# CTPLab/Tera-MIND

Hardware: AMD Instinct MI355X
Metric: denoising steps/sec on 64x64x(2 stains x 2 z) patches (interior patch-steps/s) (higher is better)
Workload: dtype f32; 1 GPU; configs[1]: b=32 images x 1 interior 64x64 patch (P=1, 128 padded + 32 collage patches/step), rna_slc=4, rna_num=229, stain=all, DDPM T=50 schedule, f32, mode A (pad+patchify -> UNet -> DDPM update); parallelism=dp1 (independent patch batches)

## Files before the change

### include/teramind_hip.h

```cpp
#ifndef TERAMIND_HIP_H
#define TERAMIND_HIP_H

#include <stddef.h>
#include <stdint.h>

#ifdef __cplusplus
extern "C" {
#endif

#define TM_ABI_VERSION 1

enum {
  TM_OK = 0,
  TM_ERR_ARG = -1,
  TM_ERR_STATE = -2,
  TM_ERR_KEY = -3,
  TM_ERR_HIP = -4,
  TM_ERR_WORKSPACE = -5
};

enum { TM_DTYPE_F32 = 0, TM_DTYPE_BF16 = 1, TM_DTYPE_F16 = 2 };
enum { TM_SAMPLE_DDPM = 0, TM_SAMPLE_DDIM = 1 };

typedef struct tm_config {
// ... 154 lines not shown
                        int res_half, int N, int Cin, int Cout, int Z, int S, int ksize, int zmode, int up2,
                        int tile_variant, void* stream);

int tm_op_conv_zpair_fused_f32(const void* x_cb8, const void* w_host, const void* bias_host, const void* norm_w_host,
                               const void* scale_host, const void* shift_host, const void* res_cb8, void* a2_out,
                               void* h1_out, void* a2_sep_out, int N, int Cin, int Cout, int Z, int S, int per_image,
                               int tile_variant, void* stream);

int tm_op_conv_ups_pair_f32(const void* x_cb8, const void* w_host, const void* bias_host, void* y_cb8, int N, int Cin,
                            int Cout, int Z, int S, int tile_variant, void* stream);

int tm_op_conv_xpair_f32(const void* x_cb8, const void* w_host, const void* bias_host, void* y_cb8, const void* res_cb8,
                         int res_half, int N, int Cin, int Cout, int Z, int S, int tile_variant, void* stream);
int tm_op_conv_xquad_f32(const void* x_cb8, const void* w_host, const void* bias_host, void* y_cb8, const void* res_cb8,
                         int res_half, int N, int Cin, int Cout, int Z, int S, int tile_variant, void* stream);
int tm_op_conv_pad1_time_f32(const void* x_cb8, const void* w_host, const void* bias_host, void* y_cb8, int N, int Cin,
                             int Cout, int S, int form, int tile_variant, int iters, float* ms_out, void* stream);

int tm_op_conv1_f32(const void* x_cb8, const void* w_host, const void* bias_host, void* y_cb8, const void* res_cb8,
                    const void* gate_cb8, int x_cbtot, int x_cb0, int gate_cbtot, int gate_cb0, int gate_half, int gelu,
                    int tile_variant, int N, int Cin, int Cout, int Z, int S, int* form_out, void* stream);
int tm_conv1_form(long vox, int ntile, int tile_variant);

int tm_conv_frag_addrs(int kernel, int half, int tw, int what, int wave, int p, int ky, int kx, int sub, int* out64);

int tm_op_conv27_bf16(const void* x_cb8, const void* w_host, const void* bias_host, void* y_cb8,
                      int N, int Cin, int Cout, int S, int dtype, int waves, const void* res_h16, void* y_h16,
                      int ups, int res_half, void* stream);
int tm_op_conv27_h16_z(const void* x_cb8, const void* w_host, const void* bias_host, void* y_cb8,
                       int N, int Cin, int Cout, int S, int dtype, int waves, const void* res_h16, void* y_h16,
                       int ups, int res_half, int Z, void* stream);

// ... 135 lines not shown
```

### tera-mind_amd/_lib.py

```python
import ctypes as C
import os

_HERE = os.path.dirname(os.path.abspath(__file__))
LIB_PATH = os.environ.get("TM_LIB_PATH") or os.path.join(_HERE, "csrc", "libteramind_hip.so")

c_void_p, c_int, c_size_t, c_char_p, c_float = C.c_void_p, C.c_int, C.c_size_t, C.c_char_p, C.c_float
c_i64_p = C.POINTER(C.c_int64)


class TmConfig(C.Structure):
    _fields_ = [("patch_size", C.c_int32), ("rna_slc", C.c_int32), ("n_stain", C.c_int32),
                ("rna_num", C.c_int32), ("net_ch", C.c_int32), ("ch_mult", C.c_int32 * 4),
                ("embed_ch", C.c_int32), ("attn_res", C.c_int32), ("num_res_blocks", C.c_int32),
                ("vis_only", C.c_int32), ("dtype", C.c_int32)]


class TmStepCoefs(C.Structure):
    _fields_ = [("sqrt_recip_alphas_cumprod", c_float), ("sqrt_recipm1_alphas_cumprod", c_float),
                ("posterior_mean_coef1", c_float), ("posterior_mean_coef2", c_float),
                ("sigma", c_float), ("sqrt_alpha_bar_prev", c_float),
                ("sqrt_one_minus_alpha_bar_prev", c_float)]


class TmProfStats(C.Structure):
# ... 61 lines not shown
    "tm_op_to_cb8": (c_int, [c_void_p, c_void_p, c_int, c_int, c_int, c_int, c_int, c_void_p]),
    "tm_op_from_cb8": (c_int, [c_void_p, c_void_p, c_int, c_int, c_int, c_int, c_int, c_void_p]),
    "tm_op_conv_mfma": (c_int, [c_void_p, c_void_p, c_void_p, c_void_p] + [c_int] * 9 + [c_void_p]),
    "tm_op_conv_mfma_res": (c_int, [c_void_p, c_void_p, c_void_p, c_void_p, c_void_p] + [c_int] * 10 + [c_void_p]),
    "tm_op_conv1_f32": (c_int, [c_void_p] * 6 + [c_int] * 12 + [C.POINTER(c_int), c_void_p]),
    "tm_conv1_form": (c_int, [C.c_long, c_int, c_int]),
    "tm_conv_frag_addrs": (c_int, [c_int] * 9 + [c_void_p]),
    "tm_op_conv27_bf16": (c_int, [c_void_p, c_void_p, c_void_p, c_void_p] + [c_int] * 6 + [c_void_p] * 2 + [c_int] * 2 + [c_void_p]),
    "tm_op_conv27_fused": (c_int, [c_void_p] * 7 + [c_int] * 7 + [c_void_p]),
    "tm_op_conv27_h16_z": (c_int, [c_void_p, c_void_p, c_void_p, c_void_p] + [c_int] * 6 + [c_void_p] * 2 + [c_int] * 3 + [c_void_p]),
    "tm_op_conv27_fused_z": (c_int, [c_void_p] * 7 + [c_int] * 8 + [c_void_p]),
    "tm_op_conv_zpair_fused_f32": (c_int, [c_void_p] * 10 + [c_int] * 7 + [c_void_p]),
    "tm_op_conv_ups_pair_f32": (c_int, [c_void_p] * 4 + [c_int] * 6 + [c_void_p]),
    "tm_op_conv_xpair_f32": (c_int, [c_void_p] * 5 + [c_int] * 7 + [c_void_p]),
    "tm_op_conv_xquad_f32": (c_int, [c_void_p] * 5 + [c_int] * 7 + [c_void_p]),
    "tm_op_conv_pad1_time_f32": (c_int, [c_void_p] * 4 + [c_int] * 7 + [C.POINTER(c_float), c_void_p]),
    "tm_op_conv27_time":(c_int, [c_int] * 10 + [c_void_p, c_void_p]),
    "tm_op_conv1_bf16": (c_int, [c_void_p, c_void_p, c_void_p, c_void_p] + [c_int] * 8 + [c_void_p] * 4),
    "tm_op_conv1_h16_gate": (c_int, [c_void_p, c_void_p, c_void_p, c_void_p] + [c_int] * 8 + [c_void_p] * 3 + [c_int] * 3 + [c_void_p]),
    "tm_op_conv1_concat": (c_int, [c_void_p, c_void_p, c_void_p, c_int, c_void_p, c_void_p, c_void_p] + [c_int] * 8 + [c_void_p]),
    "tm_op_prep_h16": (c_int, [c_void_p] * 3 + [c_int] * 7 + [c_void_p, c_int, c_int, c_void_p, c_void_p, C.c_long] +
                       [c_int] * 4 + [c_void_p, c_void_p, c_int, c_void_p, c_void_p]),
    "tm_op_prep_f32": (c_int, [c_void_p] * 3 + [c_int] * 7 + [c_void_p, c_int, c_int, c_void_p, c_void_p, C.c_long] +
                       [c_int] * 4 + [c_void_p, c_void_p, c_int, c_void_p, c_void_p]),
    "tm_op_prep_form": (c_int, [c_void_p] * 3 + [c_int] * 9 + [c_void_p, c_int, c_int, c_int, c_void_p, c_void_p, C.c_long] +
                        [c_int] * 5 + [c_void_p, c_void_p, c_int, c_int, c_void_p, c_void_p]),
    "tm_op_stem": (c_int, [c_void_p] * 4 + [c_int] * 6 + [c_void_p]),
    "tm_op_head": (c_int, [c_void_p] * 4 + [c_int] * 6 + [c_void_p]),
    "tm_op_time_embed": (c_int, [c_void_p] * 7 + [c_int] * 3 + [c_void_p]),
    "tm_op_emb_all": (c_int, [c_void_p] * 4 + [c_int] * 3 + [c_void_p]),
    "tm_op_prep_train": (c_int, [c_void_p] * 5 + [c_float, c_int, c_void_p] + [c_int] * 4 + [c_void_p]),
# ... 68 lines not shown
```

### tera-mind_amd/csrc/tm_kernels.h

```cpp
#pragma once
#include <hip/hip_runtime.h>
#include <stdint.h>

#include <vector>

#include "../../include/teramind_hip.h"

namespace tmk {

struct TV {
  float* p = nullptr;
  int N = 0, C = 0, Cb = 0, Z = 0, H = 0, W = 0;
  long nstride = 0;
  long plane() const { return (long)Z * H * W * 8; }
  TV blocks(int cb0, int ncb) const {
    TV v = *this;
    v.p = p + (long)cb0 * plane();
    v.Cb = ncb;
    v.C = ncb * 8;
    return v;
  }
};
inline TV cb8_view(void* p, int N, int C, int Z, int H, int W) {
  TV t;
// ... 38 lines not shown

enum { EPI_NONE = 0, EPI_GELU = 1, EPI_UP2 = 2 };
enum { ZM_PAD1 = 0, ZM_INPLANE = 1, ZM_VALID = 2,
       ZM_UPS = 3 };
struct ConvLaunch {
  TV x;
  ConvW w;
  TV y;
  const TV* res = nullptr;
  const TV* gate = nullptr;
  int flags = 0;
  int tile_variant = 0;
  int gate_half = 0;
  int res_half = 0;
  int zmode = ZM_PAD1;
  int fuse_norm = 0;
  const float *norm_w = nullptr, *mod_scale = nullptr, *mod_shift = nullptr;
  float inv_c = 0.f;
  long mod_stride = 0;
  int per_image = 1;
  TV a2;
};
hipError_t launch_conv_mfma(const ConvLaunch& L, hipStream_t s);
int conv_tile(int form, long ovox, int ntile, int S, int tile_variant);
int conv_frag_addrs(int kernel, int half, int tw, int what, int wv, int p, int ky, int kx, int sub, int* out);
int conv1_form(long vox, int ntile, int tile_variant);

struct TVH {
  uint16_t* p = nullptr;
  int N = 0, C = 0, Cb = 0, Z = 0, H = 0, W = 0;
  long nstride = 0;
  TVH blocks(int cb0, int ncb) const {
    TVH t = *this;
    t.p = p + (long)cb0 * Z * H * W * 8;
    t.Cb = ncb; t.C = ncb * 8;
    return t;
  }
};
struct ConvLaunchH {
  TVH x;
// ... 298 lines not shown
```

### tera-mind_amd/csrc/tm_kernels.hip

```cpp
#include "tm_conv_pair.h"

#include <stdlib.h>
#include <string.h>

#include <type_traits>

namespace tmk {

template <int NZI, int WM, int TW, bool UPS = false>
struct C3Geo {
  static constexpr int TW_ = TW;
  static constexpr int MV = 4 * WM * 32;
  static constexpr int TR = (MV / TW < TW) ? (MV / TW) : TW;
  static constexpr int NPB = MV / (TR * TW);
  static constexpr int HR = TR + 2, HC = TW + 2;
  static constexpr int XV = NPB * NZI * HR * HC;
  static constexpr int XPIECES = XV * 2;
  static constexpr int PX = (XPIECES + 255) / 256;
  static constexpr int TZ = UPS ? 4 : 9;
  static constexpr int NTAP = TZ * NZI;
  static constexpr int WFLOATS = NTAP * 512;
  static constexpr int WPIECES = WFLOATS / 4;
  static constexpr int PW = (WPIECES + 255) / 256;
  static constexpr int TAPS_TOTAL = (NZI == 1) ? 9 : 3 * TZ;
// ... 638 lines not shown
    }
#pragma unroll
    for (int z = 0; z < 2; ++z)
#pragma unroll
      for (int par = 0; par < 2; ++par) {
        f32x16 o[1][1];
        o[0][0] = acc[0][par] + acc[1 + z][par];
        asm volatile("" : "+v"(o[0][0]));
        const int ooff[1] = {ooff0 >= 0 ? ooff0 + (z * S * S + par) * 8 : -1};
        __builtin_amdgcn_sched_barrier(0);
        conv_epilogue<1, 1>(a, o, nte, h, on, ooff, 2 * S);
      }
  }
}

template <int HALF, int TW>
struct XQGeo {
  static constexpr int TW_ = TW;
  static constexpr int NW = HALF ? 4 : 8;
  static constexpr int MG = 16 * NW;
  static constexpr int GW = TW / 4;
  static constexpr int TR = (MG / GW < TW) ? (MG / GW) : TW;
  static constexpr int NPB = MG / (TR * GW);
  static constexpr int HR = TR + 2;
  static constexpr int XP = NPB * HR * GW;
  static constexpr int XITEMS = XP * 2;
  static_assert(XP % 8 == 0, "whole groups of eight staging items (tm_conv_frag.h)");
  static constexpr int WTAP = 256;
  static constexpr int WSLOT = 18 * WTAP;
  static constexpr int KP = (18 + NW - 1) / NW;
  static constexpr int LDS_BYTES = (2 * WSLOT + 18 * XP * 8) * 4;
  static_assert(2 * WSLOT * 4 <= 65536 && LDS_BYTES <= 160 * 1024, "LDS-DMA destinations below 64 KiB, the CU's LDS");
};
TM_HD constexpr int xq_lane_group(int tw, int i32) { return tw == 8 ? conv_lane_voxel(16, i32) : i32; }
template <class G>
TM_HD constexpr int xq_xtap(int q, int ky) { return q * G::XP * 8 + conv_frag_off(ky * G::GW, 0, G::XP); }

template <int HALF, int TW>
__global__ __launch_bounds__(HALF ? 256 : 512, 2) void conv3d_xquad(ConvArgs a) {
  using G = XQGeo<HALF, TW>;
  static_assert(G::XITEMS <= 64 * G::NW, "one staging item per thread");
  extern __shared__ __attribute__((aligned(16))) float lds[];
  float* lw = lds;

  const int tid = threadIdx.x;
  const int lane = tid & 63, wv = tid >> 6;
  const int i32 = lane & 31, h = lane >> 5;

  const int S = a.S;
  const ConvTile t = conv_tile_of<TW, G::TR, false, false>(a);
  const int nt = t.nt, pg = t.pg, tr = t.tr, tc = t.tc;

  long xoff = -1;
  bool okl = false, okr = false;
  if (tid < G::XITEMS) {
    const int half = conv_stage_half(tid);
    int v = conv_stage_row(tid);
    const int j = v % G::GW; v /= G::GW;
    const int hr = v % G::HR;
    const int ps = v / G::HR;
    const int n = pg * G::NPB + ps;
    const int y = tr * G::TR + hr - 1, x = tc * TW + 4 * j;
    if (n < a.N && y >= 0 && y < S) {
      xoff = (long)n * a.x_nstride + ((long)y * S + x) * 8 + half * 4;
      okl = x > 0;
      okr = x + 4 < S;
    }
  }
  const long zplane = (long)S * S * 8;
  int xw = 2 * G::WSLOT + conv_frag_off(conv_stage_row(tid), conv_stage_half(tid), G::XP);
  asm volatile("" : "+v"(xw));

  const int gt = wv >> 1;
  const int qh = wv & 1;
  int xb[3], on[1], ooff0;
  {
    const ConvLane l = conv_lane_of<G::TR, G::GW, G::HR * G::GW, G::GW, G::XP>(gt * 32 + xq_lane_group(TW, i32), h, 0, 0);
#pragma unroll
    for (int p = 0; p < 3; ++p) {
      xb[p] = (2 * G::WSLOT + (p * 6 + 3 * qh) * G::XP * 8 + l.xb) / 4;
      asm volatile("" : "+v"(xb[p]));
    }
    const int n = pg * G::NPB + l.ps;
    on[0] = n;
    const int y = tr * G::TR + l.r, x = tc * TW + 4 * l.c;
    ooff0 = n < a.N ? (y * S + x) * 8 : -1;
  }
  const int wb = 3 * qh * G::WTAP + conv_frag_off(i32, h, 32);

  f32x16 acc[3][3];
  clear_acc(acc);

  const unsigned lw_lds = (unsigned)(size_t)(__attribute__((address_space(3))) float*)lw;
  const rsrc_words wrs = weight_rsrc<true>(a.w + (long)nt * a.Cbi * 3 * G::WSLOT, a.Cbi * 3 * G::WSLOT * 4);
  const int wvo = lane * 16;
// ... 4 lines not shown

  f32x4 xr[2][6];
  const f32x4 zero4 = {0.f, 0.f, 0.f, 0.f};
  auto load_x = [&](int cb) {
    const float* xp = a.x + (long)cb * a.x_plane;
#pragma unroll
    for (int z = 0; z < 2; ++z) {
      const float* b = xp + xoff + z * zplane;
      xr[z][0] = okl ? *(const f32x4*)(b - 8) : zero4;
#pragma unroll
      for (int c = 0; c < 4; ++c) xr[z][1 + c] = xoff >= 0 ? *(const f32x4*)(b + 8 * c) : zero4;
      xr[z][5] = okr ? *(const f32x4*)(b + 32) : zero4;
    }
  };
  auto put_t = [&](int p, const f32x4 (&d)[6]) __attribute__((always_inline)) {
    float* o = lds + xw + p * 6 * G::XP * 8;
    const f32x4 e42 = d[4] - d[2];
    *(f32x4*)(o) = (4.f * d[0] - 5.f * d[2]) + d[4];
    *(f32x4*)(o + G::XP * 8) = (d[3] + d[4]) - 4.f * (d[1] + d[2]);
    *(f32x4*)(o + 2 * G::XP * 8) = 4.f * (d[1] - d[2]) - (d[3] - d[4]);
    *(f32x4*)(o + 3 * G::XP * 8) = 2.f * (d[3] - d[1]) + e42;
    *(f32x4*)(o + 4 * G::XP * 8) = 2.f * (d[1] - d[3]) + e42;
    *(f32x4*)(o + 5 * G::XP * 8) = (4.f * d[1] - 5.f * d[3]) + d[5];
  };

  load_x(0);
#pragma unroll
  for (int k = 0; k < G::KP; ++k) issue_piece(0, k);
  auto stage = [&](int cb, auto more_c) __attribute__((always_inline)) {
    constexpr bool more = decltype(more_c)::value;
    asm volatile("s_waitcnt vmcnt(0)" ::: "memory");
    __builtin_amdgcn_s_barrier();
    asm volatile("" ::: "memory");
    if (tid < G::XITEMS) {
      put_t(2, xr[0]);
#pragma unroll
      for (int c = 0; c < 6; ++c) xr[0][c] = xr[0][c] + xr[1][c];
      put_t(0, xr[0]);
      put_t(1, xr[1]);
    }
// ... 20 lines not shown
      for (int ky = 0; ky < 3; ++ky) {
#pragma unroll
        for (int q = 0; q < 3; ++q) {
          const f32x4 wf = *(const f32x4*)(lwc + (ky * 6 + q) * G::WTAP);
          const f32x4 xf = ((const f32x4*)lds)[xb[p] + xq_xtap<G>(q, ky) / 4];
#pragma unroll
          for (int kk = 0; kk < 4; ++kk) acc[p][q] = __builtin_amdgcn_mfma_f32_32x32x2f32(wf[kk], xf[kk], acc[p][q], 0, 0, 0);
          if (ky * 3 + q < G::KP && (p < 2 || more)) issue_piece(n + 1, ky * 3 + q);
        }
      }
    }
    __builtin_amdgcn_s_setprio(0);
  };
  for (int cb = 0; cb + 1 < a.Cbi; ++cb) stage(cb, std::true_type{});
  stage(a.Cbi - 1, std::false_type{});

  const int qhu = __builtin_amdgcn_readfirstlane(qh);
#pragma unroll
  for (int p = 0; p < 3; ++p) {
    if (qhu) {
      const f32x16 sp = acc[p][0] + acc[p][1];
      acc[p][0] = acc[p][0] - acc[p][1];
      acc[p][1] = sp;
    } else {
      const f32x16 s = acc[p][1] + acc[p][2];
      acc[p][2] = acc[p][1] - acc[p][2];
      acc[p][1] = s;
    }
    asm volatile("" : "+v"(acc[p][0]), "+v"(acc[p][1]), "+v"(acc[p][2]));
  }
// ... 151 lines not shown
static bool conv_fills_chip(long vox, long tiles) { return (vox / 256) * tiles >= 512; }

int conv1_form(long vox, int ntile, int tile_variant) {
  if (tile_variant == 3) return (ntile & 1) == 0 ? 3 : 0;
  const int variant = tile_variant ? tile_variant : (conv_fills_chip(vox, ntile) ? 2 : 1);
  if (variant == 2 && (ntile & 1) == 0 && conv_fills_chip(vox, ntile / 2)) return 3;
  return variant == 2 ? 2 : 1;
}

int conv_tile(int form, long ovox, int ntile, int S, int tile_variant) {
  if (S == 4) return 1;
  if (form == CF_XQUAD) return tile_variant ? (tile_variant == 2 ? 2 : 1) : ((ovox / 1024) * 2 * ntile >= 256 ? 2 : 1);
  const long tiles = (form == CF_ZSKIP_UPS || form == CF_PAIR_UPS) ? 4L * ntile : ntile;
  const int variant = tile_variant ? tile_variant : (conv_fills_chip(ovox, tiles) ? 2 : 1);
  return variant == 2 ? 2 : 1;
}

template <void (*KERN)(ConvArgs), class G, int BLOCK = 256>
static hipError_t launch_tiled(const ConvArgs& a, long factor, hipStream_t s) {
  static DevOnce attr_once;
  if (attr_once.need()) {
    hipError_t e = hipFuncSetAttribute((const void*)KERN, hipFuncAttributeMaxDynamicSharedMemorySize, G::LDS_BYTES);
    if (e != hipSuccess) return e;
    attr_once.mark();
  }
  const long tiles = (long)(a.S / G::TW_) * (a.S / G::TR);
  const long pgs = (a.N + G::NPB - 1) / G::NPB;
  hipLaunchKernelGGL(KERN, dim3((unsigned)(pgs * tiles * factor * a.ntile)), dim3(BLOCK), G::LDS_BYTES, s, a);
  return hipGetLastError();
}
// ... 104 lines not shown
      return with_tile_width<32>(S, [&](auto tw) {
        constexpr int TW = decltype(tw)::value;
        if (L.fuse_norm) return launch_tiled<conv3d_zpair<0, TW, true>, ZPGeo<0, TW>>(a, 1, s);
        return large ? launch_tiled<conv3d_zpair<0, TW, false>, ZPGeo<0, TW>>(a, 1, s)
                     : launch_tiled<conv3d_zpair<1, TW, false>, ZPGeo<1, TW>>(a, 1, s);
      });
    case CF_PAIR_UPS:
      if (S == 4) return launch_tiled<conv3d_zpair_ups<1, 4>, ZPUGeo<1, 4>>(a, 4, s);
      return with_tile_width<32>(S, [&](auto tw) {
        constexpr int TW = decltype(tw)::value;
        return large ? launch_tiled<conv3d_zpair_ups<0, TW>, ZPUGeo<0, TW>>(a, 4, s)
                     : launch_tiled<conv3d_zpair_ups<1, TW>, ZPUGeo<1, TW>>(a, 4, s);
      });
    case CF_XQUAD:
      a.ntile = (L.w.Cout + 31) / 32;
      return with_tile_width<16>(S, [&](auto tw) {
        constexpr int TW = decltype(tw)::value;
        return large ? launch_tiled<conv3d_xquad<0, TW>, XQGeo<0, TW>, 64 * XQGeo<0, TW>::NW>(a, 1, s)
                     : launch_tiled<conv3d_xquad<1, TW>, XQGeo<1, TW>, 64 * XQGeo<1, TW>::NW>(a, 1, s);
      });
    default:
      return with_tile_width<16>(S, [&](auto tw) {
        constexpr int TW = decltype(tw)::value;
        return large ? launch_tiled<conv3d_xpair<0, TW>, XPGeo<0, TW>, 64 * XPGeo<0, TW>::NW>(a, 1, s)
                     : launch_tiled<conv3d_xpair<1, TW>, XPGeo<1, TW>, 64 * XPGeo<1, TW>::NW>(a, 1, s);
      });
  }
}

template <class G, int HALF, int TW, bool UPS>
static int zpair_frag_addrs(int what, int wv, int p, int ky, int kx, int sub, int* out) {
  constexpr int NC = HALF ? 1 : 2, KW = UPS ? 2 : 3;
  constexpr int lx = G::LDS_BYTES / 4 - 3 * G::XV * 8;
  if (p < 0 || p > 2) return -1;
// ... 19 lines not shown
  using G = XPGeo<HALF, TW>;
  if (p < 0 || p > 2 || q < 0 || q >= (what == 2 ? 4 : G::NQ) || ky < 0 || ky > (what == 2 ? 0 : 2)) return -1;
  const int pt = HALF ? 0 : (wv >> 1), ch = wv & 1, q0 = HALF ? (wv >> 1) * 2 : 0;
  for (int lane = 0; lane < 64; ++lane) {
    const int i32 = lane & 31, h = lane >> 5, tid = wv * 64 + lane;
    int a = -1;
    if (what == 0) a = q0 * 512 + conv_w_off(ch * 32 + i32, 4 * h) + (ky * 4 + q) * 512;
    else if (what == 1)
      a = 2 * G::WSLOT + q0 * G::XP * 8 + conv_lane_of<G::TR, G::PWD, G::HR * G::PWD, G::PWD, G::XP>(pt * 32 + i32, h, 0, 0).xb + xp_xtap<G>(p, q, ky);
    else if (tid < G::XITEMS)
      a = 2 * G::WSLOT + conv_frag_off(conv_stage_row(tid), conv_stage_half(tid), G::XP) + (p * 4 + q) * G::XP * 8;
    out[lane] = a < 0 ? -1 : a * 4;
  }
  return 0;
}
template <int HALF, int TW>
static int xquad_frag_addrs(int what, int wv, int p, int ky, int q, int* out) {
  using G = XQGeo<HALF, TW>;
  if (wv >= G::NW || p < 0 || p > 2 || q < 0 || q >= (what == 2 ? 6 : 3) || ky < 0 || ky > (what == 2 ? 0 : 2)) return -1;
  const int gt = wv >> 1, qh = wv & 1;
  for (int lane = 0; lane < 64; ++lane) {
    const int i32 = lane & 31, h = lane >> 5, tid = wv * 64 + lane;
    int a = -1;
    if (what == 0) a = 3 * qh * G::WTAP + conv_frag_off(i32, h, 32) + (ky * 6 + q) * G::WTAP;
    else if (what == 1)
      a = 2 * G::WSLOT + (p * 6 + 3 * qh) * G::XP * 8 +
          conv_lane_of<G::TR, G::GW, G::HR * G::GW, G::GW, G::XP>(gt * 32 + xq_lane_group(TW, i32), h, 0, 0).xb + xq_xtap<G>(q, ky);
    else if (tid < G::XITEMS)
      a = 2 * G::WSLOT + conv_frag_off(conv_stage_row(tid), conv_stage_half(tid), G::XP) + (p * 6 + q) * G::XP * 8;
    out[lane] = a < 0 ? -1 : a * 4;
  }
  return 0;
}
int conv_frag_addrs(int kernel, int half, int tw, int what, int wv, int p, int ky, int kx, int sub, int* out) {
  if (!out || kernel < 0 || kernel > 4 || kernel == 3 || half < 0 || half > 1 || what < 0 || what > 2 || wv < 0 || wv > (kernel == 4 ? 7 : 3)) return -1;
  if (kernel == 4 && tw == 8) return half ? xquad_frag_addrs<1, 8>(what, wv, p, ky, kx, out) : xquad_frag_addrs<0, 8>(what, wv, p, ky, kx, out);
  if (kernel == 4 && tw == 16) return half ? xquad_frag_addrs<1, 16>(what, wv, p, ky, kx, out) : xquad_frag_addrs<0, 16>(what, wv, p, ky, kx, out);
  if (kernel == 4) return -1;
#define TM_FRAG(H, T)                                                                                              \
  if (half == H && tw == T) {                                                                                      \
    if (kernel == 0) return zpair_frag_addrs<ZPGeo<H, T>, H, T, false>(what, wv, p, ky, kx, sub, out);              \
    if (kernel == 1) return zpair_frag_addrs<ZPUGeo<H, T>, H, T, true>(what, wv, p, ky, kx, sub, out);              \
  }
  TM_FRAG(1, 4) TM_FRAG(0, 8) TM_FRAG(1, 8) TM_FRAG(0, 16) TM_FRAG(1, 16) TM_FRAG(0, 32) TM_FRAG(1, 32)
#undef TM_FRAG
  if (kernel == 2 && tw == 8) return half ? xpair_frag_addrs<1, 8>(what, wv, p, ky, kx, out) : xpair_frag_addrs<0, 8>(what, wv, p, ky, kx, out);
  if (kernel == 2 && tw == 16) return half ? xpair_frag_addrs<1, 16>(what, wv, p, ky, kx, out) : xpair_frag_addrs<0, 16>(what, wv, p, ky, kx, out);
  return -1;
}

struct PrepArgs { PrepLaunch L; };
struct PrepDropArgs { PrepLaunch L; DropRng r; };
__device__ __forceinline__ DropRng rng_of(const PrepArgs&) { return DropRng{0ull, 0u, 0u}; }
// ... 970 lines not shown
```

### tera-mind_amd/csrc/tm_ops.hip

```cpp
#include "../../include/teramind_hip.h"
#include "tm_kernels.h"

#include <algorithm>
#include <cmath>
#include <cstdint>
#include <tuple>
#include <utility>
#include <vector>
#include <string.h>

using namespace tmk;

struct DevTmp {
  std::vector<void*> ptrs;
  std::vector<hipEvent_t> events;
  hipError_t err = hipSuccess;
  const char* what = "";
  bool ordered = false;
  hipStream_t st = nullptr;
  DevTmp() = default;
  explicit DevTmp(hipStream_t stream) : ordered(true), st(stream) { keep_pool(); }
  static void keep_pool() {
    static bool done[64] = {};
    int dev = 0;
// ... 232 lines not shown
  const int rc = finish((hipStream_t)stream, launch_conv_mfma(op.L, (hipStream_t)stream), "conv_xpair (fp32)");
  return rc ? rc : conv_tile(CF_XPAIR, (long)N * Z * S * S, op.L.w.ntile, S, tile_variant);
}

static int xquad_args(const void* x, const void* w, const void* b, const void* y, int N, int Cin, int Cout, int Z, int S,
                      int tile_variant) {
  if (!x || !w || !b || !y) return fail(TM_ERR_ARG, "null argument");
  if (N < 1 || Cin < 1 || Cout < 1) return fail(TM_ERR_ARG, "N, Cin, Cout must be positive");
  if (Z != 2) return fail(TM_ERR_ARG, "the x-quad form exists at Z == 2 only (got Z = %d)", Z);
  if (S != 8 && S != 16 && S != 32 && S != 64 && S != 128) return fail(TM_ERR_ARG, "S must be 8, 16, 32, 64 or 128 (got %d)", S);
  if (tile_variant < 0 || tile_variant > 2) return fail(TM_ERR_ARG, "tile_variant must be 0 (auto), 1 or 2 (got %d)", tile_variant);
  if (conv_pick_form(3, ZM_PAD1, 2, true, ROLE_OP_XQUAD) != CF_XQUAD)
    return fail(TM_ERR_ARG, "the x-quad form is switched off (TM_CONV_XQUAD=0)");
  return TM_OK;
}
extern "C" int tm_op_conv_xquad_f32(const void* x_cb8, const void* w_host, const void* bias_host, void* y_cb8, const void* res_cb8,
                                    int res_half, int N, int Cin, int Cout, int Z, int S, int tile_variant, void* stream) {
  if (const int rc = xquad_args(x_cb8, w_host, bias_host, y_cb8, N, Cin, Cout, Z, S, tile_variant)) return rc;
  if (res_half && !res_cb8) return fail(TM_ERR_ARG, "res_half needs a residual");
  ConvOp op;
  if (const int rc = conv_op(op, CF_XQUAD, w_host, bias_host, x_cb8, y_cb8, N, Cin, Cout, Z, S, Z, S, ZM_PAD1, tile_variant, res_cb8,
                             res_half))
    return rc;
  const int rc = finish((hipStream_t)stream, launch_conv_mfma(op.L, (hipStream_t)stream), "conv_xquad (fp32)");
  return rc ? rc : conv_tile(CF_XQUAD, (long)N * Z * S * S, op.L.w.ntile, S, tile_variant);
}

extern "C" int tm_op_conv_pad1_time_f32(const void* x_cb8, const void* w_host, const void* bias_host, void* y_cb8, int N, int Cin,
                                        int Cout, int S, int form, int tile_variant, int iters, float* ms_out, void* stream) {
  if (const int rc = form == 2 ? xquad_args(x_cb8, w_host, bias_host, y_cb8, N, Cin, Cout, 2, S, tile_variant)
                               : xpair_args(x_cb8, w_host, bias_host, y_cb8, N, Cin, Cout, 2, S, tile_variant))
    return rc;
  if (form < 0 || form > 2 || iters < 1 || !ms_out) return fail(TM_ERR_ARG, "form must be 0, 1 or 2, iters >= 1, ms_out non-null");
  const int cf = conv_pick_form(3, ZM_PAD1, 2, true, form == 2 ? ROLE_OP_XQUAD : form ? ROLE_OP_XPAIR : ROLE_OP);
  if (!form && cf != CF_PAIR) return fail(TM_ERR_ARG, "the pair form is switched off (TM_CONV_ZPAIR=0)");
  ConvOp op;
  if (const int rc = conv_op(op, cf, w_host, bias_host, x_cb8, y_cb8, N, Cin, Cout, 2, S, 2, S, ZM_PAD1, tile_variant)) return rc;
  hipEvent_t e0 = op.tmp.event(), e1 = op.tmp.event();
  if (op.tmp.err) return op.tmp.report();
  hipStream_t st = (hipStream_t)stream;
  for (int i = 0; i < iters; ++i) {
    HIP_TRY(hipEventRecord(e0, st));
    HIP_TRY(launch_conv_mfma(op.L, st));
    HIP_TRY(hipEventRecord(e1, st));
    HIP_TRY(hipEventSynchronize(e1));
    HIP_TRY(hipEventElapsedTime(ms_out + i, e0, e1));
  }
  return finish(st, hipSuccess, "conv_pad1_time (fp32)");
}

static bool half_gate_ok(int S) { return S >= 2 && (S & (S - 1)) == 0; }

extern "C" int tm_conv1_form(long vox, int ntile, int tile_variant) { return conv1_form(vox, ntile, tile_variant); }
extern "C" int tm_conv_frag_addrs(int kernel, int half, int tw, int what, int wave, int p, int ky, int kx, int sub, int* out64) {
  return conv_frag_addrs(kernel, half, tw, what, wave, p, ky, kx, sub, out64);
}

extern "C" int tm_op_conv1_f32(const void* x_cb8, const void* w_host, const void* bias_host, void* y_cb8, const void* res_cb8,
                               const void* gate_cb8, int x_cbtot, int x_cb0, int gate_cbtot, int gate_cb0, int gate_half, int gelu,
                               int tile_variant, int N, int Cin, int Cout, int Z, int S, int* form_out, void* stream) {
  if (!x_cb8 || !w_host || !bias_host || !y_cb8) return fail(TM_ERR_ARG, "null argument");
  if (N < 1 || Cin < 1 || Cout < 1 || Z < 1 || S < 1) return fail(TM_ERR_ARG, "N, Cin, Cout, Z, S must be positive");
  const int Cbi = (Cin + 7) / 8, Cob = (Cout + 7) / 8;
  if (x_cb0 < 0 || x_cb0 + Cbi > x_cbtot)
    return fail(TM_ERR_ARG, "x slice: blocks [%d, %d) run past the %d blocks of the tensor", x_cb0, x_cb0 + Cbi, x_cbtot);
  if (gate_half && !gate_cb8) return fail(TM_ERR_ARG, "gate_half without a gate");
  if (gate_half && !half_gate_ok(S)) return fail(TM_ERR_ARG, "gate_half: S must be a power of two >= 2 (got %d)", S);
  if (gate_cb8 && (gate_cb0 < 0 || gate_cb0 + Cob > gate_cbtot))
// ... 1248 lines not shown
```

Measured before the change: 996.8 interior patch-steps/s.

## Add software-pipelined schedule to x-quad Winograd conv kernel with double-buffered staging

Adds a PIPE variant of the x-quad 3D conv kernel that double-buffers the transformed input sets and weight slots in LDS. The next channel block's global loads, Winograd transforms and LDS-DMA weight pieces are interleaved with the current block's MFMA taps, so only one barrier is needed per z-plane step instead of several. The aim is to hide load and staging latency behind matrix math. It becomes the default for the large tile at width 16, with an env switch to turn it off, and it costs more register pressure and a more complex waitcnt schedule.

New measurement: 1011 interior patch-steps/s, median of 6. 1.5% higher.

```diff
diff --git a/include/teramind_hip.h b/include/teramind_hip.h
--- a/include/teramind_hip.h
+++ b/include/teramind_hip.h
@@ -192,8 +192,13 @@
                          int res_half, int N, int Cin, int Cout, int Z, int S, int tile_variant, void* stream);
 int tm_op_conv_xquad_f32(const void* x_cb8, const void* w_host, const void* bias_host, void* y_cb8, const void* res_cb8,
                          int res_half, int N, int Cin, int Cout, int Z, int S, int tile_variant, void* stream);
+int tm_op_conv_xquad_sched_f32(const void* x_cb8, const void* w_host, const void* bias_host, void* y_cb8, const void* res_cb8,
+                               int res_half, int N, int Cin, int Cout, int Z, int S, int tile_variant, int sched, void* stream);
+int tm_conv_xquad_lds_bytes(int half, int tw, int sched);
 int tm_op_conv_pad1_time_f32(const void* x_cb8, const void* w_host, const void* bias_host, void* y_cb8, int N, int Cin,
                              int Cout, int S, int form, int tile_variant, int iters, float* ms_out, void* stream);
+int tm_op_conv_pad1_time_sched_f32(const void* x_cb8, const void* w_host, const void* bias_host, void* y_cb8, int N, int Cin,
+                                   int Cout, int S, int form, int tile_variant, int sched, int iters, float* ms_out, void* stream);
 
 int tm_op_conv1_f32(const void* x_cb8, const void* w_host, const void* bias_host, void* y_cb8, const void* res_cb8,
                     const void* gate_cb8, int x_cbtot, int x_cb0, int gate_cbtot, int gate_cb0, int gate_half, int gelu,
diff --git a/tera-mind_amd/_lib.py b/tera-mind_amd/_lib.py
--- a/tera-mind_amd/_lib.py
+++ b/tera-mind_amd/_lib.py
@@ -99,7 +99,10 @@
     "tm_op_conv_ups_pair_f32": (c_int, [c_void_p] * 4 + [c_int] * 6 + [c_void_p]),
     "tm_op_conv_xpair_f32": (c_int, [c_void_p] * 5 + [c_int] * 7 + [c_void_p]),
     "tm_op_conv_xquad_f32": (c_int, [c_void_p] * 5 + [c_int] * 7 + [c_void_p]),
+    "tm_op_conv_xquad_sched_f32": (c_int, [c_void_p] * 5 + [c_int] * 8 + [c_void_p]),
+    "tm_conv_xquad_lds_bytes": (c_int, [c_int] * 3),
     "tm_op_conv_pad1_time_f32": (c_int, [c_void_p] * 4 + [c_int] * 7 + [C.POINTER(c_float), c_void_p]),
+    "tm_op_conv_pad1_time_sched_f32": (c_int, [c_void_p] * 4 + [c_int] * 8 + [C.POINTER(c_float), c_void_p]),
     "tm_op_conv27_time":(c_int, [c_int] * 10 + [c_void_p, c_void_p]),
     "tm_op_conv1_bf16": (c_int, [c_void_p, c_void_p, c_void_p, c_void_p] + [c_int] * 8 + [c_void_p] * 4),
     "tm_op_conv1_h16_gate": (c_int, [c_void_p, c_void_p, c_void_p, c_void_p] + [c_int] * 8 + [c_void_p] * 3 + [c_int] * 3 + [c_void_p]),
diff --git a/tera-mind_amd/csrc/tm_kernels.h b/tera-mind_amd/csrc/tm_kernels.h
--- a/tera-mind_amd/csrc/tm_kernels.h
+++ b/tera-mind_amd/csrc/tm_kernels.h
@@ -76,6 +76,7 @@
   int gate_half = 0;
   int res_half = 0;
   int zmode = ZM_PAD1;
+  int xquad_sched = -1;
   int fuse_norm = 0;
   const float *norm_w = nullptr, *mod_scale = nullptr, *mod_shift = nullptr;
   float inv_c = 0.f;
@@ -86,6 +87,7 @@
 hipError_t launch_conv_mfma(const ConvLaunch& L, hipStream_t s);
 int conv_tile(int form, long ovox, int ntile, int S, int tile_variant);
 int conv_frag_addrs(int kernel, int half, int tw, int what, int wv, int p, int ky, int kx, int sub, int* out);
+int conv_xquad_lds_bytes(int half, int tw, int sched);
 int conv1_form(long vox, int ntile, int tile_variant);
 
 struct TVH {
diff --git a/tera-mind_amd/csrc/tm_kernels.hip b/tera-mind_amd/csrc/tm_kernels.hip
--- a/tera-mind_amd/csrc/tm_kernels.hip
+++ b/tera-mind_amd/csrc/tm_kernels.hip
@@ -676,7 +676,7 @@
   }
 }
 
-template <int HALF, int TW>
+template <int HALF, int TW, int PIPE = 0>
 struct XQGeo {
   static constexpr int TW_ = TW;
   static constexpr int NW = HALF ? 4 : 8;
@@ -691,16 +691,37 @@
   static constexpr int WTAP = 256;
   static constexpr int WSLOT = 18 * WTAP;
   static constexpr int KP = (18 + NW - 1) / NW;
-  static constexpr int LDS_BYTES = (2 * WSLOT + 18 * XP * 8) * 4;
+  static constexpr int XSET = 6 * XP * 8;
+  static constexpr int NSET = PIPE ? 2 : 3;
+  static constexpr int XCH = NW * 3 * 1024;
+  static constexpr int LDS_BYTES = (2 * WSLOT + NSET * XSET > XCH ? 2 * WSLOT + NSET * XSET : XCH) * 4;
   static_assert(2 * WSLOT * 4 <= 65536 && LDS_BYTES <= 160 * 1024, "LDS-DMA destinations below 64 KiB, the CU's LDS");
+  static_assert(!PIPE || !HALF || LDS_BYTES <= 80 * 1024, "two workgroups of the small tile per CU");
 };
+template <class V>
+TM_HD V xq_transform(int q, const V (&d)[6]) {
+  switch (q) {
+    case 0: return (4.f * d[0] - 5.f * d[2]) + d[4];
+    case 1: return (d[3] + d[4]) - 4.f * (d[1] + d[2]);
+    case 2: return 4.f * (d[1] - d[2]) - (d[3] - d[4]);
+    case 3: return 2.f * (d[3] - d[1]) + (d[4] - d[2]);
+    case 4: return 2.f * (d[1] - d[3]) + (d[4] - d[2]);
+    default: return (4.f * d[1] - 5.f * d[3]) + d[5];
+  }
+}
 TM_HD constexpr int xq_lane_group(int tw, int i32) { return tw == 8 ? conv_lane_voxel(16, i32) : i32; }
 template <class G>
 TM_HD constexpr int xq_xtap(int q, int ky) { return q * G::XP * 8 + conv_frag_off(ky * G::GW, 0, G::XP); }
-
-template <int HALF, int TW>
+template <class G>
+TM_HD constexpr int xq_xfrag(int set, int qh, int lxb) { return set * G::XSET + 3 * qh * G::XP * 8 + lxb; }
+template <class G>
+TM_HD constexpr int xq_xstage(int set, int q, int item) {
+  return set * G::XSET + q * G::XP * 8 + conv_frag_off(conv_stage_row(item), conv_stage_half(item), G::XP);
+}
+
+template <int HALF, int TW, int PIPE>
 __global__ __launch_bounds__(HALF ? 256 : 512, 2) void conv3d_xquad(ConvArgs a) {
-  using G = XQGeo<HALF, TW>;
+  using G = XQGeo<HALF, TW, PIPE>;
   static_assert(G::XITEMS <= 64 * G::NW, "one staging item per thread");
   extern __shared__ __attribute__((aligned(16))) float lds[];
   float* lw = lds;
@@ -730,7 +751,7 @@
     }
   }
   const long zplane = (long)S * S * 8;
-  int xw = 2 * G::WSLOT + conv_frag_off(conv_stage_row(tid), conv_stage_half(tid), G::XP);
+  int xw = 2 * G::WSLOT + xq_xstage<G>(0, 0, tid);
   asm volatile("" : "+v"(xw));
 
   const int gt = wv >> 1;
@@ -740,7 +761,7 @@
     const ConvLane l = conv_lane_of<G::TR, G::GW, G::HR * G::GW, G::GW, G::XP>(gt * 32 + xq_lane_group(TW, i32), h, 0, 0);
 #pragma unroll
     for (int p = 0; p < 3; ++p) {
-      xb[p] = (2 * G::WSLOT + (p * 6 + 3 * qh) * G::XP * 8 + l.xb) / 4;
+      xb[p] = (2 * G::WSLOT + xq_xfrag<G>(p, qh, l.xb)) / 4;
       asm volatile("" : "+v"(xb[p]));
     }
     const int n = pg * G::NPB + l.ps;
@@ -775,16 +796,102 @@
     }
   };
   auto put_t = [&](int p, const f32x4 (&d)[6]) __attribute__((always_inline)) {
-    float* o = lds + xw + p * 6 * G::XP * 8;
-    const f32x4 e42 = d[4] - d[2];
-    *(f32x4*)(o) = (4.f * d[0] - 5.f * d[2]) + d[4];
-    *(f32x4*)(o + G::XP * 8) = (d[3] + d[4]) - 4.f * (d[1] + d[2]);
-    *(f32x4*)(o + 2 * G::XP * 8) = 4.f * (d[1] - d[2]) - (d[3] - d[4]);
-    *(f32x4*)(o + 3 * G::XP * 8) = 2.f * (d[3] - d[1]) + e42;
-    *(f32x4*)(o + 4 * G::XP * 8) = 2.f * (d[1] - d[3]) + e42;
-    *(f32x4*)(o + 5 * G::XP * 8) = (4.f * d[1] - 5.f * d[3]) + d[5];
+    float* o = lds + xw + p * G::XSET;
+#pragma unroll
+    for (int q = 0; q < 6; ++q) *(f32x4*)(o + q * G::XP * 8) = xq_transform(q, d);
   };
 
+  if constexpr (PIPE) {
+  const bool stg = tid < G::XITEMS;
+  const bool ldw = __builtin_amdgcn_readfirstlane(wv * 64 < G::XITEMS);
+  auto load_xc = [&](int cb) __attribute__((always_inline)) {
+    const float* xp = a.x + (long)cb * a.x_plane + (xoff >= 0 ? xoff : 0);
+#pragma unroll
+    for (int z = 0; z < 2; ++z) {
+      const float* b = xp + z * zplane;
+      xr[z][0] = *(const f32x4*)(okl ? b - 8 : b);
+#pragma unroll
+      for (int c = 0; c < 4; ++c) xr[z][1 + c] = *(const f32x4*)(b + 8 * c);
+      xr[z][5] = *(const f32x4*)(okr ? b + 32 : b);
+    }
+  };
+  auto mask_x = [&](int z) __attribute__((always_inline)) {
+    xr[z][0] = okl ? xr[z][0] : zero4;
+#pragma unroll
+    for (int c = 0; c < 4; ++c) xr[z][1 + c] = xoff >= 0 ? xr[z][1 + c] : zero4;
+    xr[z][5] = okr ? xr[z][5] : zero4;
+#pragma unroll
+    for (int c = 0; c < 6; ++c) asm volatile("" : "+v"(xr[z][c]));
+  };
+  int xw4 = xw / 4;
+  asm volatile("" : "+v"(xw4));
+  auto put_q = [&](int q, const f32x4 (&d)[6], int set) __attribute__((always_inline)) {
+    ((f32x4*)lds)[xw4 + set * (G::XSET / 4) + q * G::XP * 2] = xq_transform(q, d);
+  };
+  constexpr int LOADTAP = G::KP > 3 ? G::KP - 1 : 2;
+  static_assert(LOADTAP < 9, "inside the product");
+
+#pragma unroll
+  for (int k = 0; k < G::KP; ++k) lds_dma_piece<4, 18, G::NW>(lw_lds, 0, 2 * G::WSLOT, k, wvu, wvo, wrs);
+  if (ldw) load_xc(0);
+  else {
+#pragma unroll
+    for (int c = 0; c < 12; ++c) xr[c / 6][c % 6] = zero4;
+  }
+  mask_x(0);
+  if (stg) {
+#pragma unroll
+    for (int q = 0; q < 6; ++q) put_q(q, xr[0], 0);
+  }
+  auto block = [&](int cb, auto more_c) __attribute__((always_inline)) {
+    constexpr bool more = decltype(more_c)::value;
+    __builtin_amdgcn_s_setprio(1);
+#pragma unroll
+    for (int i = 0; i < 3; ++i) {
+      const int n = cb * 3 + i, par = n & 1;
+      const int p = 2 - i;
+      const bool follows = i < 2 || more;
+      if (i == 2 && more && ldw) asm volatile("s_waitcnt vmcnt(12)" ::: "memory");
+      else asm volatile("s_waitcnt vmcnt(0)" ::: "memory");
+      __builtin_amdgcn_s_waitcnt(0xC07F);
+      __builtin_amdgcn_sched_barrier(0);
+      __builtin_amdgcn_s_barrier();
+      asm volatile("" ::: "memory");
+      __builtin_amdgcn_sched_barrier(0);
+      const float* lwc = lw + par * G::WSLOT + wb;
+      const int xbn = xb[0] + par * (G::XSET / 4);
+      const int nsrc = (i == 2 ? cb * 3 + 5 : cb * 3 + p - 1) * G::WSLOT;
+#pragma unroll
+      for (int ky = 0; ky < 3; ++ky) {
+#pragma unroll
+        for (int q = 0; q < 3; ++q) {
+          const int tap = ky * 3 + q;
+          const f32x4 wf = *(const f32x4*)(lwc + (ky * 6 + q) * G::WTAP);
+          const f32x4 xf = ((const f32x4*)lds)[xbn + xq_xtap<G>(q, ky) / 4];
+          if (follows) {
+            if (tap == 0 && i != 1) mask_x(i == 0 ? 1 : 0);
+            if (i == 1) {
+              if (tap == 0) {
+#pragma unroll
+                for (int c = 0; c < 6; ++c) xr[0][c] = xr[0][c] + xr[1][c];
+              }
+              if (tap < 3 && stg) { put_q(2 * tap, xr[0], par ^ 1); put_q(2 * tap + 1, xr[0], par ^ 1); }
+            } else if (tap < 6 && stg) {
+              put_q(tap, i == 0 ? xr[1] : xr[0], par ^ 1);
+            }
+            if (tap < G::KP) lds_dma_piece<4, 18, G::NW>(lw_lds, (par ^ 1) * G::WSLOT, nsrc, tap, wvu, wvo, wrs);
+            if (i == 1 && more && tap == LOADTAP && ldw) load_xc(cb + 1);
+          }
+#pragma unroll
+          for (int kk = 0; kk < 4; ++kk) acc[p][q] = __builtin_amdgcn_mfma_f32_32x32x2f32(wf[kk], xf[kk], acc[p][q], 0, 0, 0);
+        }
+      }
+    }
+    __builtin_amdgcn_s_setprio(0);
+  };
+  for (int cb = 0; cb + 1 < a.Cbi; ++cb) block(cb, std::true_type{});
+  block(a.Cbi - 1, std::false_type{});
+  } else {
   load_x(0);
 #pragma unroll
   for (int k = 0; k < G::KP; ++k) issue_piece(0, k);
@@ -835,6 +942,7 @@
   };
   for (int cb = 0; cb + 1 < a.Cbi; ++cb) stage(cb, std::true_type{});
   stage(a.Cbi - 1, std::false_type{});
+  }
 
   const int qhu = __builtin_amdgcn_readfirstlane(qh);
 #pragma unroll
@@ -1016,6 +1124,14 @@
   const long tiles = (form == CF_ZSKIP_UPS || form == CF_PAIR_UPS) ? 4L * ntile : ntile;
   const int variant = tile_variant ? tile_variant : (conv_fills_chip(ovox, tiles) ? 2 : 1);
   return variant == 2 ? 2 : 1;
+}
+
+static bool xquad_pipe_default(bool half, int tw) {
+  static const bool on = [] {
+    const char* v = getenv("TM_CONV_XQUAD_PIPE");
+    return !(v && atoi(v) == 0);
+  }();
+  return on && !half && tw == 16;
 }
 
 template <void (*KERN)(ConvArgs), class G, int BLOCK = 256>
@@ -1150,10 +1266,14 @@
       });
     case CF_XQUAD:
       a.ntile = (L.w.Cout + 31) / 32;
+      if (L.xquad_sched < -1 || L.xquad_sched > 1) return hipErrorInvalidValue;
       return with_tile_width<16>(S, [&](auto tw) {
         constexpr int TW = decltype(tw)::value;
-        return large ? launch_tiled<conv3d_xquad<0, TW>, XQGeo<0, TW>, 64 * XQGeo<0, TW>::NW>(a, 1, s)
-                     : launch_tiled<conv3d_xquad<1, TW>, XQGeo<1, TW>, 64 * XQGeo<1, TW>::NW>(a, 1, s);
+        if (L.xquad_sched < 0 ? xquad_pipe_default(!large, TW) : L.xquad_sched == 1)
+          return large ? launch_tiled<conv3d_xquad<0, TW, 1>, XQGeo<0, TW, 1>, 64 * XQGeo<0, TW, 1>::NW>(a, 1, s)
+                       : launch_tiled<conv3d_xquad<1, TW, 1>, XQGeo<1, TW, 1>, 64 * XQGeo<1, TW, 1>::NW>(a, 1, s);
+        return large ? launch_tiled<conv3d_xquad<0, TW, 0>, XQGeo<0, TW, 0>, 64 * XQGeo<0, TW, 0>::NW>(a, 1, s)
+                     : launch_tiled<conv3d_xquad<1, TW, 0>, XQGeo<1, TW, 0>, 64 * XQGeo<1, TW, 0>::NW>(a, 1, s);
       });
     default:
       return with_tile_width<16>(S, [&](auto tw) {
@@ -1203,29 +1323,39 @@
   }
   return 0;
 }
-template <int HALF, int TW>
-static int xquad_frag_addrs(int what, int wv, int p, int ky, int q, int* out) {
-  using G = XQGeo<HALF, TW>;
+template <int HALF, int TW, int PIPE>
+static int xquad_frag_addrs(int what, int wv, int p, int ky, int q, int set, int* out) {
+  using G = XQGeo<HALF, TW, PIPE>;
   if (wv >= G::NW || p < 0 || p > 2 || q < 0 || q >= (what == 2 ? 6 : 3) || ky < 0 || ky > (what == 2 ? 0 : 2)) return -1;
+  if (set < 0 || set >= G::NSET) return -1;
   const int gt = wv >> 1, qh = wv & 1;
   for (int lane = 0; lane < 64; ++lane) {
     const int i32 = lane & 31, h = lane >> 5, tid = wv * 64 + lane;
     int a = -1;
     if (what == 0) a = 3 * qh * G::WTAP + conv_frag_off(i32, h, 32) + (ky * 6 + q) * G::WTAP;
     else if (what == 1)
-      a = 2 * G::WSLOT + (p * 6 + 3 * qh) * G::XP * 8 +
-          conv_lane_of<G::TR, G::GW, G::HR * G::GW, G::GW, G::XP>(gt * 32 + xq_lane_group(TW, i32), h, 0, 0).xb + xq_xtap<G>(q, ky);
+      a = 2 * G::WSLOT + xq_xtap<G>(q, ky) +
+          xq_xfrag<G>(set, qh, conv_lane_of<G::TR, G::GW, G::HR * G::GW, G::GW, G::XP>(gt * 32 + xq_lane_group(TW, i32), h, 0, 0).xb);
     else if (tid < G::XITEMS)
-      a = 2 * G::WSLOT + conv_frag_off(conv_stage_row(tid), conv_stage_half(tid), G::XP) + (p * 6 + q) * G::XP * 8;
+      a = 2 * G::WSLOT + xq_xstage<G>(set, q, tid);
     out[lane] = a < 0 ? -1 : a * 4;
   }
   return 0;
 }
+int conv_xquad_lds_bytes(int half, int tw, int sched) {
+  if (half < 0 || half > 1 || (tw != 8 && tw != 16) || sched < 0 || sched > 1) return -1;
+  if (sched) return half ? (tw == 8 ? XQGeo<1, 8, 1>::LDS_BYTES : XQGeo<1, 16, 1>::LDS_BYTES) : (tw == 8 ? XQGeo<0, 8, 1>::LDS_BYTES : XQGeo<0, 16, 1>::LDS_BYTES);
+  return half ? (tw == 8 ? XQGeo<1, 8, 0>::LDS_BYTES : XQGeo<1, 16, 0>::LDS_BYTES) : (tw == 8 ? XQGeo<0, 8, 0>::LDS_BYTES : XQGeo<0, 16, 0>::LDS_BYTES);
+}
 int conv_frag_addrs(int kernel, int half, int tw, int what, int wv, int p, int ky, int kx, int sub, int* out) {
-  if (!out || kernel < 0 || kernel > 4 || kernel == 3 || half < 0 || half > 1 || what < 0 || what > 2 || wv < 0 || wv > (kernel == 4 ? 7 : 3)) return -1;
-  if (kernel == 4 && tw == 8) return half ? xquad_frag_addrs<1, 8>(what, wv, p, ky, kx, out) : xquad_frag_addrs<0, 8>(what, wv, p, ky, kx, out);
-  if (kernel == 4 && tw == 16) return half ? xquad_frag_addrs<1, 16>(what, wv, p, ky, kx, out) : xquad_frag_addrs<0, 16>(what, wv, p, ky, kx, out);
-  if (kernel == 4) return -1;
+  const bool xq = kernel == 4 || kernel == 5;
+  if (!out || kernel < 0 || kernel > 5 || kernel == 3 || half < 0 || half > 1 || what < 0 || what > 2 || wv < 0 || wv > (xq ? 7 : 3)) return -1;
+  if (kernel == 4 && tw == 8) return half ? xquad_frag_addrs<1, 8, 0>(what, wv, p, ky, kx, p, out) : xquad_frag_addrs<0, 8, 0>(what, wv, p, ky, kx, p, out);
+  if (kernel == 4 && tw == 16) return half ? xquad_frag_addrs<1, 16, 0>(what, wv, p, ky, kx, p, out) : xquad_frag_addrs<0, 16, 0>(what, wv, p, ky, kx, p, out);
+  if (kernel == 5 && what == 0 && sub != 0) return -1;
+  if (kernel == 5 && tw == 8) return half ? xquad_frag_addrs<1, 8, 1>(what, wv, p, ky, kx, sub, out) : xquad_frag_addrs<0, 8, 1>(what, wv, p, ky, kx, sub, out);
+  if (kernel == 5 && tw == 16) return half ? xquad_frag_addrs<1, 16, 1>(what, wv, p, ky, kx, sub, out) : xquad_frag_addrs<0, 16, 1>(what, wv, p, ky, kx, sub, out);
+  if (xq) return -1;
 #define TM_FRAG(H, T)                                                                                              \
   if (half == H && tw == T) {                                                                                      \
     if (kernel == 0) return zpair_frag_addrs<ZPGeo<H, T>, H, T, false>(what, wv, p, ky, kx, sub, out);              \
diff --git a/tera-mind_amd/csrc/tm_ops.hip b/tera-mind_amd/csrc/tm_ops.hip
--- a/tera-mind_amd/csrc/tm_ops.hip
+++ b/tera-mind_amd/csrc/tm_ops.hip
@@ -270,28 +270,40 @@
     return fail(TM_ERR_ARG, "the x-quad form is switched off (TM_CONV_XQUAD=0)");
   return TM_OK;
 }
-extern "C" int tm_op_conv_xquad_f32(const void* x_cb8, const void* w_host, const void* bias_host, void* y_cb8, const void* res_cb8,
-                                    int res_half, int N, int Cin, int Cout, int Z, int S, int tile_variant, void* stream) {
+static int xquad_op(const void* x_cb8, const void* w_host, const void* bias_host, void* y_cb8, const void* res_cb8, int res_half, int N,
+                    int Cin, int Cout, int Z, int S, int tile_variant, int sched, void* stream) {
   if (const int rc = xquad_args(x_cb8, w_host, bias_host, y_cb8, N, Cin, Cout, Z, S, tile_variant)) return rc;
   if (res_half && !res_cb8) return fail(TM_ERR_ARG, "res_half needs a residual");
   ConvOp op;
   if (const int rc = conv_op(op, CF_XQUAD, w_host, bias_host, x_cb8, y_cb8, N, Cin, Cout, Z, S, Z, S, ZM_PAD1, tile_variant, res_cb8,
                              res_half))
     return rc;
+  op.L.xquad_sched = sched;
   const int rc = finish((hipStream_t)stream, launch_conv_mfma(op.L, (hipStream_t)stream), "conv_xquad (fp32)");
   return rc ? rc : conv_tile(CF_XQUAD, (long)N * Z * S * S, op.L.w.ntile, S, tile_variant);
 }
-
-extern "C" int tm_op_conv_pad1_time_f32(const void* x_cb8, const void* w_host, const void* bias_host, void* y_cb8, int N, int Cin,
-                                        int Cout, int S, int form, int tile_variant, int iters, float* ms_out, void* stream) {
+extern "C" int tm_op_conv_xquad_f32(const void* x_cb8, const void* w_host, const void* bias_host, void* y_cb8, const void* res_cb8,
+                                    int res_half, int N, int Cin, int Cout, int Z, int S, int tile_variant, void* stream) {
+  return xquad_op(x_cb8, w_host, bias_host, y_cb8, res_cb8, res_half, N, Cin, Cout, Z, S, tile_variant, -1, stream);
+}
+extern "C" int tm_op_conv_xquad_sched_f32(const void* x_cb8, const void* w_host, const void* bias_host, void* y_cb8, const void* res_cb8,
+                                          int res_half, int N, int Cin, int Cout, int Z, int S, int tile_variant, int sched, void* stream) {
+  if (sched != 0 && sched != 1) return fail(TM_ERR_ARG, "sched must be 0 (four barriers) or 1 (pipelined) (got %d)", sched);
+  return xquad_op(x_cb8, w_host, bias_host, y_cb8, res_cb8, res_half, N, Cin, Cout, Z, S, tile_variant, sched, stream);
+}
+
+static int pad1_time(const void* x_cb8, const void* w_host, const void* bias_host, void* y_cb8, int N, int Cin, int Cout, int S, int form,
+                     int tile_variant, int sched, int iters, float* ms_out, void* stream) {
   if (const int rc = form == 2 ? xquad_args(x_cb8, w_host, bias_host, y_cb8, N, Cin, Cout, 2, S, tile_variant)
                                : xpair_args(x_cb8, w_host, bias_host, y_cb8, N, Cin, Cout, 2, S, tile_variant))
     return rc;
   if (form < 0 || form > 2 || iters < 1 || !ms_out) return fail(TM_ERR_ARG, "form must be 0, 1 or 2, iters >= 1, ms_out non-null");
+  if (sched < -1 || sched > 1 || (sched >= 0 && form != 2)) return fail(TM_ERR_ARG, "sched must be -1, or 0 | 1 with form 2 (got %d)", sched);
   const int cf = conv_pick_form(3, ZM_PAD1, 2, true, form == 2 ? ROLE_OP_XQUAD : form ? ROLE_OP_XPAIR : ROLE_OP);
   if (!form && cf != CF_PAIR) return fail(TM_ERR_ARG, "the pair form is switched off (TM_CONV_ZPAIR=0)");
   ConvOp op;
   if (const int rc = conv_op(op, cf, w_host, bias_host, x_cb8, y_cb8, N, Cin, Cout, 2, S, 2, S, ZM_PAD1, tile_variant)) return rc;
+  op.L.xquad_sched = sched;
   hipEvent_t e0 = op.tmp.event(), e1 = op.tmp.event();
   if (op.tmp.err) return op.tmp.report();
   hipStream_t st = (hipStream_t)stream;
@@ -304,10 +316,20 @@
   }
   return finish(st, hipSuccess, "conv_pad1_time (fp32)");
 }
+extern "C" int tm_op_conv_pad1_time_f32(const void* x_cb8, const void* w_host, const void* bias_host, void* y_cb8, int N, int Cin,
+                                        int Cout, int S, int form, int tile_variant, int iters, float* ms_out, void* stream) {
+  return pad1_time(x_cb8, w_host, bias_host, y_cb8, N, Cin, Cout, S, form, tile_variant, -1, iters, ms_out, stream);
+}
+extern "C" int tm_op_conv_pad1_time_sched_f32(const void* x_cb8, const void* w_host, const void* bias_host, void* y_cb8, int N, int Cin,
+                                              int Cout, int S, int form, int tile_variant, int sched, int iters, float* ms_out,
+                                              void* stream) {
+  return pad1_time(x_cb8, w_host, bias_host, y_cb8, N, Cin, Cout, S, form, tile_variant, sched, iters, ms_out, stream);
+}
 
 static bool half_gate_ok(int S) { return S >= 2 && (S & (S - 1)) == 0; }
 
 extern "C" int tm_conv1_form(long vox, int ntile, int tile_variant) { return conv1_form(vox, ntile, tile_variant); }
+extern "C" int tm_conv_xquad_lds_bytes(int half, int tw, int sched) { return conv_xquad_lds_bytes(half, tw, sched); }
 extern "C" int tm_conv_frag_addrs(int kernel, int half, int tw, int what, int wave, int p, int ky, int kx, int sub, int* out64) {
   return conv_frag_addrs(kernel, half, tw, what, wave, p, ky, kx, sub, out64);
 }
```
